# ishine/usdm

Measured on AMD Instinct MI355X. Metric: end-to-end real-time factor + LLM tokens/sec, 10 s utterance, 7B TP=1/8, higher is better.
Workload: dtype bf16; 1 GPU; full pipeline, one 10 s utterance: XLS-R tokenizer -> Mistral-7B (3 greedy rounds) -> Token-Voicebox 63 NFE (Heun, CFG, 3 s prompt) -> BigVGAN; wave_samples=160000, mel_frames=861, output_samples=220416, parallelism=tp1 (LLM) + replicas, tp_comm=none, voicebox=replica (CFG batch 2 on every rank)

## Files before the change

### include/usdm_hip.h

```cpp
#ifndef USDM_HIP_H_
#define USDM_HIP_H_
#include <stdint.h>

#ifdef __cplusplus
extern "C" {
#endif

typedef void* usdm_stream_t;

enum { USDM_BF16 = 0, USDM_F32 = 1 };
enum { USDM_ACT_NONE = 0, USDM_ACT_GELU = 1, USDM_ACT_SWIGLU = 3, USDM_ACT_TANH = 4, USDM_ACT_LOGCLAMP = 5  };
enum { USDM_EPI_PLAIN = 0, USDM_EPI_QKV_HEADS = 1 };

const char* usdm_last_error(void);
int usdm_abi_version(void);

typedef struct usdm_gemm_args {
  int32_t dtype;
  int32_t M, N;
  int32_t taps, Kc;
  const void* A;
  int64_t lda;
  int32_t rowsA;
  int32_t a_row_mul, a_row_off, a_row_step;
  int64_t a_tap_stride;
  const void* W;
  int64_t ldw;
  int32_t groups, batch;
  int64_t a_gstride;
  int64_t w_gstride;
  int64_t a_bstride;
  int32_t c_gcol;
  int64_t c_bstride;
  const float* bias;
  float alpha;
  int32_t act;
  int32_t round_bf16;
  const void* residual;
  int32_t res_dtype;
  int64_t ldr;
  void* C32;
  void* C16;
  int64_t ldc;
  int32_t c_row_mul, c_row_off;
  int32_t transpose_out;
  int32_t epi;
  int32_t qkv_S, qkv_Spad, qkv_H, qkv_D;
  void *qkv_q, *qkv_k, *qkv_v;
  int32_t split_k; int64_t c_split_stride;
  float* stats_out;
  const float* ln_stats; int32_t ln_nt, ln_mode, ln_C; float ln_eps;
  const float* ln_c; const float* ln_gamma; const float* ln_beta;
  int32_t* ln_guard; float ln_guard_ratio;
  int32_t tile_sel;
} usdm_gemm_args;

int usdm_gemm(const usdm_gemm_args* args, usdm_stream_t stream);
int usdm_gemm_tile_for(const usdm_gemm_args* args);

typedef struct usdm_norm_args {
  const void* x; int32_t x_dtype; int64_t ldx;
  const void* res; int32_t res_dtype; int64_t ldr;
  const float* gamma; const float* beta; float eps;
  int32_t rows, C;
  int32_t rms, act, round_bf16, premask;
  const int32_t* valid_len; int32_t rows_per_batch;
  void* out32; void* out16; int64_t ldo;
  void* sum32; void* sum16; int64_t lds;
  const float* res2; int32_t n_res2; int64_t res2_stride;
} usdm_norm_args;

int usdm_norm(const usdm_norm_args* args, usdm_stream_t stream);

typedef struct usdm_snake_args {
  const float* x; int64_t ldx;
  int32_t T, C, Creal, L;
  const float* alpha; const float* beta; int32_t logscale;
  float fup[12]; float fdn[12];
  float* out32; void* out16; int64_t ldo;
} usdm_snake_args;
int usdm_aa_snake(const usdm_snake_args* args, usdm_stream_t stream);

int usdm_sum3_scale(const float* a, const float* b, const float* c, float scale, int64_t n,
                    float* out32, void* out16_bf16, usdm_stream_t stream);

int usdm_cf_to_cl(const float* x, int32_t B, int32_t C, int32_t T, int32_t Cpad, float scale, float shift,
                  float* out32, void* out16_bf16, usdm_stream_t stream);

typedef struct usdm_attn_args {
  int32_t mode, dh, B, Hq, Hkv, Sq, Skv, Skv_alloc, q_pos0, alibi_col0_zero;
  float scale;
  int32_t head_order;
  const void* q; int64_t q_bs, q_hs, q_rs;
  const void* k; int64_t k_bs, k_hs, k_rs;
  const void* vt; int64_t v_bs, v_hs, v_ds;
  void* o; int64_t o_bs, o_rs;
  const int32_t* kv_len;
  const float* slopes;
  int32_t window;
  int32_t variant;
} usdm_attn_args;
int usdm_attention(const usdm_attn_args* args, usdm_stream_t stream);

typedef struct usdm_vb_input_args {
  const int64_t* ids;
  const float* y;
  const float* cond;
  const void* table;
  int32_t B_in, dup, S, E, F, null_id, use_cond;
  void* out; int64_t ldo;
  int32_t out_dtype;
} usdm_vb_input_args;
int usdm_vb_build_input(const usdm_vb_input_args* args, usdm_stream_t stream);

int usdm_softmax_alibi(float* x, int32_t rows, int32_t rows_per_batch, int32_t nheads, int32_t n, int32_t npad, int64_t ldrow,
                       int32_t ldseg, const float* slopes, const int32_t* kv_len, int32_t col0_zero, usdm_stream_t stream);

int usdm_vb_time_token(const float* t, int32_t t_stride, const float* freqs, int32_t Bx, int32_t H,
                       int64_t rows_per_batch, float* h32, void* h16_bf16, usdm_stream_t stream);

typedef struct usdm_vb_solver_args {
  const float* vout;
  const float* z; float* v1; const float* eps; const float* cond;
  float* z_in; float* z_commit; float* t_cur;
  int32_t B, F, S, P, cfg, mode, t_count;
  float gs, dt, c_eps, c_cond, t_next;
} usdm_vb_solver_args;
int usdm_vb_solver_step(const usdm_vb_solver_args* args, usdm_stream_t stream);

int usdm_mask_time(float* x32, void* x16_bf16, int32_t B, int32_t T, int32_t C, int32_t layout, const int32_t* valid_len,
                   int32_t off, usdm_stream_t stream);

int usdm_copy_bytes(void* dst, const void* src, int64_t nbytes, usdm_stream_t stream);

int usdm_process_unit(const int64_t* units, int32_t n, int32_t rep, int32_t hop, int64_t* out, int32_t nframes,
                      usdm_stream_t stream);

typedef struct usdm_gemv_args {
  const void* W; int64_t ldw; int32_t N, K;
  const void* x;
  const float* norm_w; float eps;
  int32_t act, round_bf16;
  const void* residual;
  void* y16; float* y32;
  const uint8_t* ban; float* part_val; int32_t* part_idx;
  int32_t idx_offset;
  const float* x_delta; void* x_out;
  const int32_t* skip;
  const struct usdm_p2p_dev* p2p; int32_t p2p_site, p2p_mode;
  const float* mrg_pm; const float* mrg_pl; const float* mrg_po; int32_t mrg_ns;
  unsigned long long* cmb_gran; int32_t* cmb_err; int32_t cmb_timeout_ms;
  int32_t resident;
} usdm_gemv_args;
int usdm_gemv(const usdm_gemv_args* args, usdm_stream_t stream);
int usdm_gemv_nblocks(int32_t N, int32_t act);

int usdm_gemv_threads(const usdm_gemv_args* args);

typedef struct usdm_gemv_batch_args {
  usdm_gemv_args g;
  int32_t nb;
  int64_t x_bs, y_bs, res_bs;
  int32_t part_bs;
  int32_t form;
  float* ks_part; int32_t* ks_cnt; int64_t ks_part_floats;
} usdm_gemv_batch_args;
int64_t usdm_gemv_batch_ks_floats(int32_t N, int32_t K);
int usdm_gemv_batch(const usdm_gemv_batch_args* args, usdm_stream_t stream);

typedef struct usdm_gemv_fp8_args {
  usdm_gemv_batch_args b;
  const int8_t* row_exp;
} usdm_gemv_fp8_args;
int usdm_gemv_fp8(const usdm_gemv_fp8_args* args, usdm_stream_t stream);
int usdm_gemv_fp8_mfma(const usdm_gemv_fp8_args* args, usdm_stream_t stream);
int usdm_dequant_fp8(const void* q, const int8_t* row_exp, int32_t N, int32_t K, int64_t ldq, void* out, int64_t ldo,
                     usdm_stream_t stream);
int usdm_sizeof_gemv_fp8_args(void);

typedef struct usdm_gemv_mxfp4_args {
  usdm_gemv_batch_args b;
  const uint8_t* scales;
  int64_t lds;
} usdm_gemv_mxfp4_args;
int usdm_gemv_mxfp4(const usdm_gemv_mxfp4_args* args, usdm_stream_t stream);
int usdm_dequant_mxfp4(const void* codes, int64_t ldw, const uint8_t* scales, int64_t lds, int32_t N, int32_t K, void* out,
                       int64_t ldo, usdm_stream_t stream);
int usdm_sizeof_gemv_mxfp4_args(void);

typedef struct usdm_decode_state {
  int32_t* next_token;
  int32_t* out_tokens;
  int32_t* step;
  int32_t* pos;
  int32_t max_out, id_offset, advance_pos;
  int32_t batch;
  int32_t* done; const int32_t* eos;
} usdm_decode_state;
int usdm_argmax_final(const float* part_val, const int32_t* part_idx, int32_t nparts,
                      const usdm_decode_state* st, const void* embed_table_bf16, int32_t Hd, void* h_out_bf16,
                      usdm_stream_t stream);
int usdm_argmax_final_seg(const float* part_val, const int32_t* part_idx, int32_t nparts, int32_t nseg, int64_t seg_stride,
                          const usdm_decode_state* st, const void* embed_table, int32_t Hd, void* h_out, usdm_stream_t stream);

typedef struct usdm_sample_params {
  float temperature; int32_t top_k; float top_p;
  float min_p;
  uint64_t seed;
} usdm_sample_params;
typedef struct usdm_sample_args {
  const float* logits; int32_t V;
  float temperature; int32_t top_k; float top_p;
  uint64_t seed;
  float* probs_out;
  const usdm_sample_params* dev_params;
  int64_t logits_bs;
  float min_p;
} usdm_sample_args;
int usdm_sample_final(const usdm_sample_args* args, const usdm_decode_state* st, const void* embed_table_bf16, int32_t Hd,
                      void* h_out_bf16, usdm_stream_t stream);
int usdm_sample_final_seg(const usdm_sample_args* args, int32_t nseg, int64_t seg_stride, int32_t seg_len, const usdm_decode_state* st,
                          const void* embed_table_bf16, int32_t Hd, void* h_out_bf16, usdm_stream_t stream);

typedef struct usdm_logprob_args {
  const float* logits; int32_t V; int32_t K;
  int64_t logits_bs;
  float* tok_lp; int32_t* tok_rank; int32_t* top_id; float* top_lp;
  int64_t tok_bs, top_bs;
  int32_t* count;
} usdm_logprob_args;
int usdm_logprobs(const usdm_logprob_args* args, const usdm_decode_state* st, usdm_stream_t stream);
int usdm_logprobs_seg(const usdm_logprob_args* args, int32_t nseg, int64_t seg_stride, int32_t seg_len, const usdm_decode_state* st,
                      usdm_stream_t stream);
int usdm_sizeof_logprob_args(void);

typedef struct usdm_prompt_logprob_args {
  const float* logits; int32_t V; int32_t K;
  int64_t logits_bs;
  const int64_t* ids;
  int32_t n_ids;
  int32_t row0, rows;
  float* tok_lp; int32_t* tok_rank; int32_t* top_id; float* top_lp;
} usdm_prompt_logprob_args;
int usdm_prompt_logprobs(const usdm_prompt_logprob_args* args, usdm_stream_t stream);
int usdm_prompt_logprobs_seg(const usdm_prompt_logprob_args* args, int32_t nseg, int64_t seg_stride, int32_t seg_len,
                             usdm_stream_t stream);
int usdm_sizeof_prompt_logprob_args(void);

typedef struct usdm_penalty_params { float repetition, frequency, presence; int32_t reserved; } usdm_penalty_params;
typedef struct usdm_penalty_args {
  float* logits; int32_t V;
  int64_t logits_bs;
  int32_t* table;
  int64_t table_bs;
  const usdm_penalty_params* dev_params;
  int32_t* count;
} usdm_penalty_args;
int usdm_penalize(const usdm_penalty_args* args, const usdm_decode_state* st, usdm_stream_t stream);
int usdm_penalize_seg(const usdm_penalty_args* args, int32_t nseg, int64_t seg_stride, int32_t seg_len, const usdm_decode_state* st,
                      usdm_stream_t stream);
int usdm_penalty_params_init(usdm_penalty_params* out, float repetition, float frequency, float presence);
int usdm_sizeof_penalty_args(void);
int usdm_sizeof_penalty_params(void);

typedef struct usdm_logit_edit_params { int32_t ngram, prompt_len, n_bias, reserved; } usdm_logit_edit_params;
typedef struct usdm_logit_edit_args {
  float* logits; int32_t V;
  int64_t logits_bs;
  const usdm_logit_edit_params* dev_params;
  const int32_t* bias_id; const float* bias_val;
  int32_t bias_max;
  int64_t bias_bs;
  const int32_t* prompt;
  int32_t prompt_max;
  int64_t prompt_bs;
} usdm_logit_edit_args;
int usdm_logit_edit(const usdm_logit_edit_args* args, const usdm_decode_state* st, usdm_stream_t stream);
int usdm_logit_edit_seg(const usdm_logit_edit_args* args, int32_t nseg, int64_t seg_stride, int32_t seg_len, const usdm_decode_state* st,
                        usdm_stream_t stream);
int usdm_sizeof_logit_edit_args(void);
int usdm_sizeof_logit_edit_params(void);

#define USDM_BEAM_MAX_KC 32
typedef struct usdm_beam_args {
  const float* logits; int32_t V;
  int64_t logits_bs;
  float* score;
  int32_t* parent;
  int32_t nlive, n_eos;
  const int32_t* eos;
  float* log_score; int32_t* log_token; int32_t* log_parent;
  int32_t log_rows;
  float* cand_score; int32_t* cand_index;
} usdm_beam_args;
int usdm_beam_step(const usdm_beam_args* args, const usdm_decode_state* st, const void* embed_table_bf16, int32_t Hd, void* h_out_bf16,
                   usdm_stream_t stream);
int usdm_sizeof_beam_args(void);

typedef struct usdm_kv_reorder_args {
  void* base[4]; int64_t slot_bytes[4]; int32_t row_bytes[4];
  int32_t n_arrays, nblk, ctx_max, B;
  const int32_t* parent; const int32_t* lo; const int32_t* pos;
} usdm_kv_reorder_args;
int usdm_kv_reorder(const usdm_kv_reorder_args* args, usdm_stream_t stream);
int usdm_sizeof_kv_reorder_args(void);

int usdm_embed_rows(const void* table, const int64_t* ids, const int32_t* next_token, int32_t n, int32_t Hd,
                    void* out, usdm_stream_t stream);

typedef struct usdm_rope_args {
// ... 145 lines not shown
```

### usdm_amd/csrc/gemv_launch.h

```cpp
#pragma once
#include "gemv_common.h"

namespace {
struct gemv_sel { int rw, nwv; bool glu; int grid; int res; };

static int gemv_pick_rw(int nout, bool glu) {
  const int ncand = glu ? 2 : 4;
  const int cands[4] = {glu ? 2 : 4, glu ? 1 : 3, 2, 1};
  int best = cands[ncand - 1];
  double best_score = -1.0;
  for (int c = 0; c < ncand; ++c) {
    const int rw = cands[c];
    const int blocks = cdiv(nout, 4 * rw);
    const double eff = (blocks / 256.0) / (double)((blocks + 255) / 256);
    if (blocks >= 1024 && eff >= 0.9) return rw;
    const double score = eff * (blocks >= 512 ? 1.0 : 0.5 + blocks / 1024.0);
    if (score > best_score) { best_score = score; best = rw; }
  }
  return best;
}

static gemv_sel gemv_select(const usdm_gemv_args& a, bool batched) {
  const bool glu = a.act == USDM_ACT_SWIGLU;
  const int nout = glu ? a.N / 2 : a.N;
  const int rows_per_cu = nout % 256 == 0 ? nout / 256 : 0;
  const gemv_sel wide16{1, 16, false, 256}, wide12{2, 12, false, 256};
  if (!batched && (a.mrg_po || a.p2p_mode)) return rows_per_cu == 16 ? wide16 : gemv_sel{1, 4, false, cdiv(nout, 4)};
  if (!glu && !a.part_val && rows_per_cu == 16) return wide16;
  if (!glu && !a.part_val && rows_per_cu == 24) return wide12;
  if (!batched && glu && (a.resident != 0 || (nout % 14 == 0 && (nout / 14) % 512 == 0)))
    return gemv_sel{2, 7, true, cdiv(nout, 14), a.resident < 0 ? 0 : a.resident > 0 ? a.resident : 0x7fffffff};
  const int rw = a.part_val ? 4 : gemv_pick_rw(nout, glu);
  return gemv_sel{rw, 4, glu, cdiv(nout, 4 * rw)};
}

enum { GEMV_PLAIN = 1, GEMV_BATCH = 2, GEMV_MRG = 4, GEMV_CMB = 8 };
#define USDM_GEMV_SHAPES(X)                                   \
  X(1, false, 16, GEMV_PLAIN | GEMV_BATCH | GEMV_MRG | GEMV_CMB) \
  X(2, false, 12, GEMV_PLAIN | GEMV_BATCH)                    \
  X(2, true, 7, GEMV_PLAIN)                                   \
  X(4, false, 4, GEMV_PLAIN | GEMV_BATCH)                     \
  X(3, false, 4, GEMV_PLAIN | GEMV_BATCH)                     \
  X(2, false, 4, GEMV_PLAIN | GEMV_BATCH)                     \
  X(1, false, 4, GEMV_PLAIN | GEMV_BATCH | GEMV_MRG)          \
  X(2, true, 4, GEMV_PLAIN | GEMV_BATCH)                      \
  X(1, true, 4, GEMV_PLAIN | GEMV_BATCH)
template <int FORM, class LAUNCH>
static bool gemv_dispatch(const gemv_sel& s, LAUNCH&& launch) {
#define USDM_GEMV_CASE(RW, GLU, NWV, FORMS)                                      \
  if constexpr (((FORMS) & FORM) != 0)                                           \
    if (s.rw == RW && s.glu == GLU && s.nwv == NWV) {                            \
      launch(gemv_ic<RW>{}, gemv_ic<GLU>{}, gemv_ic<NWV>{});                     \
      return true;                                                               \
    }
  USDM_GEMV_SHAPES(USDM_GEMV_CASE)
#undef USDM_GEMV_CASE
  return false;
}

static int gemv_no_instantiation(const gemv_sel& s) {
  usdm_set_error("%s: no instantiation for %d rows per wave, GLU %d, %d waves", __FILE__, s.rw, (int)s.glu, s.nwv);
  return 1;
}

static int gemv_check_shape(const char* who, const usdm_gemv_args& a, const char* x_noun) {
  USDM_CHECK_ARG(a.N > 0 && a.K > 0 && a.K % 8 == 0 && a.ldw % 8 == 0 && a.ldw >= a.K, "%s: bad N/K/ldw", who);
  USDM_CHECK_ARG(a.K <= 16384, "%s: K too large for the LDS-resident %s", who, x_noun);
  USDM_CHECK_ARG(a.act != USDM_ACT_SWIGLU || a.N % 32 == 0, "%s: swiglu needs N %% 32 == 0", who);
  return 0;
}
static int gemv_check_outputs(const char* who, const usdm_gemv_args& a) {
  USDM_CHECK_ARG(a.y16 || a.y32 || a.part_val, "%s: no output", who);
  USDM_CHECK_ARG(!a.part_val || (a.part_idx && a.act != USDM_ACT_SWIGLU), "%s: part_idx missing / lm_head mode is not GLU", who);
  return 0;
}
}
```

### usdm_amd/csrc/llm_k.hip

```cpp
#include "common.h"
#include <stdlib.h>
#include <utility>
#include "../../include/usdm_hip.h"
#include "gemv_launch.h"
#include "attn_merge.h"
#include "p2p.h"
#include "pick_commit.h"

#ifndef USDM_GEMV_X_FIRST
#define USDM_GEMV_X_FIRST 1
#endif
#ifndef USDM_GEMV_RES_PREFETCH
#define USDM_GEMV_RES_PREFETCH 1
#endif
namespace {
#ifdef USDM_GEMV_TRACE
__device__ unsigned long long g_gemv_trace[8192 * 8];
#define GTR(i) do { if (threadIdx.x == 0 && blockIdx.x < 8192) g_gemv_trace[blockIdx.x * 8 + (i)] = wall_clock64(); } while (0)
#else
#define GTR(i) do { } while (0)
#endif


template <int RW, bool GLU, int NWV, bool MRG = false, bool P2P = false, bool CMB = false, bool FP8 = false, class... FMT>
__global__ __launch_bounds__(NWV * 64) void gemv_kernel(const usdm_gemv_args a, FMT... fmt) {
  typedef typename gemv_fmt<FP8>::wvec wvec;
  constexpr bool MX4 = gemv_is_mx4<FMT...>::value;
  static_assert((FP8 || MX4) == (sizeof...(FMT) == 1) && !(FP8 && MX4), "FP8 takes the row exponents, MXFP4 the block scales");
  static_assert(!(FP8 || MX4) || (!MRG && !P2P && !CMB), "the FP8 / MXFP4 weight formats have the plain single-GPU forms only");
  constexpr int NTH = NWV * 64;
  constexpr int NR = GLU ? 2 * RW : RW;
  constexpr int UNR = gemv_ring_depth(NR, FP8, MX4);
  extern __shared__ __attribute__((aligned(16))) char smem[];
  bf16_t* xs = (bf16_t*)smem;
  __shared__ float red[NWV];
  __shared__ float sv[NWV];
  __shared__ int si[NWV];
  const int tid = threadIdx.x, lane = tid & 63, wave = tid >> 6;
  const int skipv = a.skip ? *a.skip : 0;
  unsigned p2p_epoch = 0u;
  bool p2p_failed = false;
  if constexpr (P2P) { p2p_epoch = p2p_load_epoch(a.p2p); p2p_failed = p2p_load_err(a.p2p) != 0u; }
  GTR(0);
  const int K = a.K;
  const int Kpad = (K + 511) & ~511;
  const int nit = Kpad >> 9;

  const int rows_per_block = NWV * RW;
  const int ob = blockIdx.x * rows_per_block + wave * RW;
  const wvec* wp[NR];
  float wsc[NR];
  const unsigned* wsp[MX4 ? NR : 1];
#pragma unroll
  for (int j = 0; j < NR; ++j) {
    int r;
    if (GLU) {
      const int o = ob + (j % RW);
      r = (o >> 4) * 32 + (o & 15) + (j >= RW ? 16 : 0);
    } else {
      r = ob + j;
    }
    r = r < a.N ? r : a.N - 1;
    if constexpr (FP8) {
      wp[j] = (const wvec*)((const uint8_t*)a.W + (int64_t)r * a.ldw) + lane;
      wsc[j] = fp8_row_scale(gemv_row_exp(fmt...)[r]);
    } else if constexpr (MX4) {
      const gemv_mx4 m = gemv_mx4_fmt(fmt...);
      wp[j] = (const u32x4*)((const uint8_t*)a.W + (int64_t)r * a.ldw) + lane;
      wsp[j] = (const unsigned*)(m.scales + (int64_t)r * m.lds) + (lane >> 2);
    } else {
      wp[j] = (const u32x4*)((const bf16_t*)a.W + (int64_t)r * a.ldw) + lane;
    }
  }
  const int ngr = (nit + 3) >> 2;
  const bool tail_ok = ((nit - 1) << 9) + lane * 8 < K;
  bool active = true;
  if (a.part_val && a.ban) {
    const int wb = blockIdx.x * rows_per_block;
    bool wg_active = false;
    for (int r = wb; r < wb + rows_per_block && r < a.N; ++r) wg_active |= (a.ban[r] == 0);
    if (!wg_active) {
      if (tid == 0) { a.part_val[blockIdx.x] = -INFINITY; a.part_idx[blockIdx.x] = 0x7fffffff; }
      if (a.y32 && tid < rows_per_block && wb + tid < a.N) a.y32[wb + tid] = -INFINITY;
      return;
    }
    active = false;
#pragma unroll
    for (int j = 0; j < NR; ++j)
      if (ob + j < a.N) active |= (a.ban[ob + j] == 0);
    active = __builtin_amdgcn_readfirstlane(active);
  }
  auto wload = [&](int j, int it) -> wvec {
    if (!active) return wvec{};
    const wvec* p = (it == nit - 1 && !tail_ok) ? wp[j] - lane : wp[j] + it * 64;
    return __builtin_nontemporal_load(p);
  };
  unsigned short resraw[GLU ? 1 : NR];
  if constexpr (!GLU && USDM_GEMV_RES_PREFETCH) {
    const bf16_t* rbase = a.residual ? (const bf16_t*)a.residual : (const bf16_t*)a.W;
#pragma unroll
    for (int j = 0; j < NR; ++j) resraw[j] = rbase[min(ob + j, a.N - 1)];
  }
  constexpr bool EARLY = USDM_GEMV_X_FIRST && !CMB && !MRG;
  const int i0 = tid * 8;
  u32x4 x0 = {0u, 0u, 0u, 0u}, ge0v = x0, ge1v = x0;
  if constexpr (EARLY) {
    const int ic = min(i0, K - 8);
    const float* gp0 = a.norm_w ? a.norm_w + ic : (const float*)a.x;
    const float* gp1 = a.norm_w ? gp0 + 4 : gp0;
    asm volatile("global_load_dwordx4 %0, %1, off" : "=v"(x0) : "v"((const bf16_t*)a.x + ic) : "memory");
    asm volatile("global_load_dwordx4 %0, %1, off" : "=v"(ge0v) : "v"(gp0) : "memory");
    asm volatile("global_load_dwordx4 %0, %1, off" : "=v"(ge1v) : "v"(gp1) : "memory");
  }
  wvec ring[NR][UNR];
  unsigned rsc[MX4 ? NR : 1][MX4 ? UNR : 1];
#pragma unroll
  for (int u = 0; u < UNR; ++u)
#pragma unroll
    for (int j = 0; j < NR; ++j) {
      if constexpr (MX4) {
        const int g = u < ngr ? u : 0;
        ring[j][u] = __builtin_nontemporal_load(wp[j] + g * 64);
        rsc[j][u] = __builtin_nontemporal_load(wsp[j] + g * 16);
      } else {
        const bool real = active && u < nit;
        const wvec* p = real ? ((u == nit - 1 && !tail_ok) ? wp[j] - lane : wp[j] + u * 64) : wp[j] - lane;
        ring[j][u] = __builtin_nontemporal_load(p);
      }
    }
  GTR(1);
  if constexpr (EARLY) {
    constexpr int NY = (MX4 ? 2 : 1) * UNR * NR;
    asm volatile("s_waitcnt vmcnt(%3)" : "+v"(x0), "+v"(ge0v), "+v"(ge1v) : "n"(NY));
  }
  if (skipv) return;
  const float4 ge0 = __builtin_bit_cast(float4, ge0v), ge1 = __builtin_bit_cast(float4, ge1v);
  const bf16_t* xg = (const bf16_t*)a.x;
  auto with_delta = [&](u32x4 v, int i, bool publish) -> u32x4 {
    if (a.x_delta) {
      const float4 d0 = *(const float4*)(a.x_delta + i), d1 = *(const float4*)(a.x_delta + i + 4);
      const float dl[8] = {d0.x, d0.y, d0.z, d0.w, d1.x, d1.y, d1.z, d1.w};
#pragma unroll
      for (int e = 0; e < 4; ++e)
        v[e] = pack_bf2(bf2f(v[e] & 0xffff) + round_bf(dl[2 * e]), bf2f(v[e] >> 16) + round_bf(dl[2 * e + 1]));
      if (publish && a.x_out && blockIdx.x == 0) *(u32x4*)((bf16_t*)a.x_out + i) = v;
    }
    return v;
  };
  auto ldx = [&](int i, bool publish) -> u32x4 { return with_delta(*(const u32x4*)(xg + i), i, publish); };
  const int iloop = EARLY ? i0 + NTH * 8 : i0;
  if (a.norm_w) {
    float ss = 0.f;
    u32x4 v0 = x0;
    if constexpr (EARLY) {
      if (i0 < K) {
        v0 = with_delta(x0, i0, false);
#pragma unroll
        for (int e = 0; e < 4; ++e) {
          const float lo = bf2f(v0[e] & 0xffff), hi = bf2f(v0[e] >> 16);
          ss += lo * lo + hi * hi;
        }
      }
    }
    for (int i = iloop; i < K; i += NTH * 8) {
      const u32x4 v = ldx(i, false);
#pragma unroll
// ... 309 lines not shown
  const int i0 = tid * 8;
  u32x4 x0 = {0u, 0u, 0u, 0u}, ge0v = x0, ge1v = x0;
  {
    const int ic = min(i0, K - 8);
    const float* gp0 = a.norm_w ? a.norm_w + ic : (const float*)a.x;
    const float* gp1 = a.norm_w ? gp0 + 4 : gp0;
    asm volatile("global_load_dwordx4 %0, %1, off" : "=v"(x0) : "v"((const bf16_t*)a.x + ic) : "memory");
    asm volatile("global_load_dwordx4 %0, %1, off" : "=v"(ge0v) : "v"(gp0) : "memory");
    asm volatile("global_load_dwordx4 %0, %1, off" : "=v"(ge1v) : "v"(gp1) : "memory");
  }
  u32x4 ring[NR][UNR];
  if constexpr (TPW > 0) {
    static_assert(NIT == 0 || (NIT >= UNR && NIT % UNR == 0), "slot u = iteration u of every tile");
    gemv_for<UNR>([&](auto U) { gemv_for<NR>([&](auto J) { aload(ring[J.value][U.value], wp[J.value], U); }); });
  } else {
#pragma unroll
    for (int u = 0; u < UNR; ++u)
#pragma unroll
      for (int j = 0; j < NR; ++j) ring[j][u] = u < nit ? wload(wp[j], u) : __builtin_nontemporal_load((const u32x4*)wp[j]);
  }
  GTR(1);
  asm volatile("s_waitcnt vmcnt(%3)" : "+v"(x0), "+v"(ge0v), "+v"(ge1v) : "n"(UNR * NR));
  if (skipv) return;
  const float4 ge0 = __builtin_bit_cast(float4, ge0v), ge1 = __builtin_bit_cast(float4, ge1v);
  const bf16_t* xg = (const bf16_t*)a.x;
  const int iloop = i0 + NTH * 8;
  if (a.norm_w) {
    float ss = 0.f;
    if (i0 < K) {
#pragma unroll
      for (int e = 0; e < 4; ++e) {
        const float lo = bf2f(x0[e] & 0xffff), hi = bf2f(x0[e] >> 16);
        ss += lo * lo + hi * hi;
      }
    }
    for (int i = iloop; i < K; i += NTH * 8) {
      const u32x4 v = *(const u32x4*)(xg + i);
#pragma unroll
      for (int e = 0; e < 4; ++e) {
        const float lo = bf2f(v[e] & 0xffff), hi = bf2f(v[e] >> 16);
        ss += lo * lo + hi * hi;
      }
    }
    ss = wave_sum(ss);
    if (lane == 0) red[wave] = ss;
    __syncthreads();
    float tot = 0.f;
#pragma unroll
    for (int w = 0; w < NWV; ++w) tot += red[w];
    const float rstd = rsqrtf(tot / (float)K + a.eps);
    auto normed = [&](u32x4 v, float4 g0, float4 g1) -> u32x4 {
      const float gw[8] = {g0.x, g0.y, g0.z, g0.w, g1.x, g1.y, g1.z, g1.w};
      u32x4 o;
#pragma unroll
      for (int e = 0; e < 4; ++e) {
        const float lo = bf2f(v[e] & 0xffff), hi = bf2f(v[e] >> 16);
        o[e] = pack_bf2(round_bf(round_bf(lo * rstd) * gw[2 * e]), round_bf(round_bf(hi * rstd) * gw[2 * e + 1]));
      }
      return o;
    };
    if (i0 < Kpad) *(u32x4*)(xs + i0) = i0 < K ? normed(x0, ge0, ge1) : u32x4{0, 0, 0, 0};
    for (int i = iloop; i < Kpad; i += NTH * 8) {
      u32x4 o = {0, 0, 0, 0};
      if (i < K) o = normed(*(const u32x4*)(xg + i), *(const float4*)(a.norm_w + i), *(const float4*)(a.norm_w + i + 4));
      *(u32x4*)(xs + i) = o;
    }
  } else {
    if (i0 < Kpad) *(u32x4*)(xs + i0) = i0 < K ? x0 : u32x4{0, 0, 0, 0};
    for (int i = iloop; i < Kpad; i += NTH * 8) {
      u32x4 v = {0, 0, 0, 0};
      if (i < K) v = *(const u32x4*)(xg + i);
      *(u32x4*)(xs + i) = v;
    }
  }
  __syncthreads();
  GTR(2);

  float acc[NR];
  const char* wn[NR];
  auto finish = [&](int t) {
#pragma unroll
    for (int j = 0; j < NR; ++j) acc[j] = wave_sum(acc[j]);
    if (t < 4) GTR(3 + t);
    if (lane == 0) {
      const int ob = (blockIdx.x + t * gridDim.x) * TILE + wave * RW;
#pragma unroll
      for (int j = 0; j < RW; ++j) {
        const int o = ob + j;
        if (2 * o >= a.N) continue;
        const float r = gemv_swiglu_value(acc[j], acc[j + RW], a.round_bf16);
        if (a.y16) ((bf16_t*)a.y16)[o] = f2bf(r);
        if (a.y32) a.y32[o] = r;
      }
    }
#pragma unroll
    for (int j = 0; j < NR; ++j) wp[j] = wn[j];
  };
  if constexpr (TPW > 0) {
    u32x4 xv = *(const u32x4*)(xs + lane * 8);
    gemv_for<TPW>([&](auto T) {
      constexpr int t = decltype(T)::value;
      constexpr bool has_next = t + 1 < TPW;
#pragma unroll
      for (int j = 0; j < NR; ++j) {
        acc[j] = 0.f;
        wn[j] = has_next ? row_ptr(t + 1, j) : wp[j];
      }
      gemv_for<NIT>([&](auto IT) {
        constexpr int it = decltype(IT)::value, u = it % UNR;
        constexpr bool refill = it + UNR < NIT || has_next;
        const u32x4 xn = *(const u32x4*)(xs + (((it + 1) % NIT) * 64 + lane) * 8);
        gemv_for<NR>([&](auto J) {
          constexpr int j = decltype(J)::value;
          constexpr int younger = refill ? NR * UNR - 1 : NR * UNR - 1 - ((it - (NIT - UNR)) * NR + j);
          asm volatile("s_waitcnt vmcnt(%1)" : "+v"(ring[j][u]) : "n"(younger) : "memory");
          acc[j] = dot8(ring[j][u], xv, acc[j]);
          if constexpr (it + UNR < NIT) aload(ring[j][u], wp[j], gemv_ic<it + UNR>{});
          else if constexpr (has_next) aload(ring[j][u], wn[j], gemv_ic<u>{});
        });
        xv = xn;
      });
      finish(t);
    });
  } else {
    const int ntiles = (a.N / 2 + TILE - 1) / TILE;
    const int ntl = (ntiles - (int)blockIdx.x + (int)gridDim.x - 1) / (int)gridDim.x;
    for (int t = 0; t < ntl; ++t) {
      const bool has_next = t + 1 < ntl;
#pragma unroll
      for (int j = 0; j < NR; ++j) {
        acc[j] = 0.f;
        wn[j] = has_next ? row_ptr(t + 1, j) : wp[j];
      }
      for (int it0 = 0; it0 < nit; it0 += UNR) {
#pragma unroll
        for (int u = 0; u < UNR; ++u) {
          const int it = it0 + u;
          if (it < nit) {
            const u32x4 xv = *(const u32x4*)(xs + (it * 64 + lane) * 8);
#pragma unroll
            for (int j = 0; j < NR; ++j) {
              acc[j] = dot8(ring[j][u], xv, acc[j]);
              const bool own = it + UNR < nit;
              if (own || has_next) ring[j][u] = wload(own ? wp[j] : wn[j], own ? it + UNR : u);
            }
          }
        }
      }
      finish(t);
    }
  }
}

__global__ void argmax_final_kernel(const float* pv, const int* pi, int nparts, int nseg, int64_t seg_stride, usdm_decode_state st,
                                    const bf16_t* E, int Hd, bf16_t* h_out) {
  __shared__ float sv[256];
  __shared__ int si[256];
  __shared__ int s_tok;
  const int b = blockIdx.x;
  if (st.done && st.done[b]) return;
  pv += (int64_t)b * nparts; pi += (int64_t)b * nparts;
  float bv = -INFINITY;
  int bi = PICK_NO_ID;
  for (int sg = 0; sg < nseg; ++sg)
    for (int i = threadIdx.x; i < nparts; i += 256) {
      const float v = pv[sg * seg_stride + i];
      const int id = pi[sg * seg_stride + i];
      if (pick_better(v, id, bv, bi)) { bv = v; bi = id; }
    }
  pick_block_best<256>(sv, si, bv, bi);
  if (threadIdx.x == 0) {
    const int tok = (si[0] == PICK_NO_ID ? 0 : si[0]) + st.id_offset;
    pick_commit(st, b, st.step[b], tok);
    s_tok = tok;
  }
  if (E) {
    __syncthreads();
    pick_embed_row<256>(E, s_tok, Hd, h_out + (int64_t)b * Hd);
  }
}

__global__ void embed_kernel(const bf16_t* E, const int64_t* ids, const int* next_token, int n, int Hd, bf16_t* out) {
  const int r = blockIdx.x;
  const int64_t id = ids ? ids[r] : (int64_t)(*next_token);
  const u32x4* src = (const u32x4*)(E + id * Hd);
  u32x4* dst = (u32x4*)(out + (int64_t)r * Hd);
  for (int i = threadIdx.x; i < Hd / 8; i += blockDim.x) dst[i] = src[i];
}

__global__ void residual_add_kernel(bf16_t* h, const float* delta, int n) {
  const int i = blockIdx.x * blockDim.x + threadIdx.x;
  if (i < n) h[i] = f2bf(bf2f(h[i]) + round_bf(delta[i]));
}
}

static int gemv_resident_count(const void* kern, int nth, size_t lds, int* out) {
  static thread_local const void* c_kern = nullptr;
  static thread_local int c_dev = -1, c_n = 0;
  static thread_local size_t c_lds = 0;
  int dev = 0;
  USDM_HIP(hipGetDevice(&dev));
  if (kern != c_kern || dev != c_dev || lds != c_lds) {
    int ncu = 0, per = 0;
    USDM_HIP(hipDeviceGetAttribute(&ncu, hipDeviceAttributeMultiprocessorCount, dev));
    USDM_HIP(hipOccupancyMaxActiveBlocksPerMultiprocessor(&per, kern, nth, lds));
    USDM_CHECK_ARG(ncu > 0 && per > 0, "usdm_gemv: the resident form does not fit a CU (%zu bytes of LDS)", lds);
    c_kern = kern; c_dev = dev; c_lds = lds; c_n = ncu * per;
  }
  *out = c_n;
  return 0;
}

static int gemv_launch_resident(const usdm_gemv_args& a, const gemv_sel& s, size_t lds, hipStream_t st, bool* launched) {
  *launched = false;
  if (a.x_delta) return 0;
  constexpr int RW = 2, NWV = 7;
  auto straight = gemv_resident_kernel<RW, NWV, 2, 8>;
  auto generic = gemv_resident_kernel<RW, NWV, 0, 0>;
  const int ntiles = s.grid;
  int n = 0;
  if (int rc = gemv_resident_count((const void*)straight, NWV * 64, lds, &n)) return rc;
  int grid = min(min(n, s.res), ntiles);
  if (grid == ntiles) return 0;
  if (a.K == 8 * 512 && ntiles == 2 * grid) {
    hipLaunchKernelGGL(straight, dim3(grid), dim3(NWV * 64), lds, st, a);
  } else {
    if (int rc = gemv_resident_count((const void*)generic, NWV * 64, lds, &n)) return rc;
    grid = min(min(n, s.res), ntiles);
    if (grid == ntiles) return 0;
    hipLaunchKernelGGL(generic, dim3(grid), dim3(NWV * 64), lds, st, a);
  }
  *launched = true;
  USDM_LAUNCH_CHECK();
  return 0;
}

template <int FORM, bool MRG, bool P2P, bool CMB, bool FP8, class... FMT>
static int gemv_launch(const usdm_gemv_args& a, hipStream_t st, FMT... fmt) {
  const size_t lds = (size_t)((a.K + 511) & ~511) * 2;
  const gemv_sel s = gemv_select(a, false);
  if constexpr (FORM == GEMV_PLAIN && !FP8 && sizeof...(FMT) == 0) {
    if (s.res > 0) {
      bool launched = false;
      if (int rc = gemv_launch_resident(a, s, lds, st, &launched)) return rc;
      if (launched) return 0;
    }
  }
  const bool found = gemv_dispatch<FORM>(s, [&](auto RW, auto GLU, auto NWV) {
    constexpr int nwv = decltype(NWV)::value;
    hipLaunchKernelGGL((gemv_kernel<decltype(RW)::value, decltype(GLU)::value != 0, nwv, MRG, P2P, CMB, FP8, FMT...>), dim3(s.grid),
                       dim3(nwv * 64), lds, st, a, fmt...);
  });
  if (!found) return gemv_no_instantiation(s);
  USDM_LAUNCH_CHECK();
  return 0;
}

extern "C" int usdm_gemv(const usdm_gemv_args* pa, usdm_stream_t stream) {
  USDM_CHECK_ARG(pa && pa->W && (pa->x || pa->mrg_po), "usdm_gemv: null args");
  const usdm_gemv_args& a = *pa;
  if (int rc = gemv_check_shape("usdm_gemv", a, "input vector")) return rc;
  if (int rc = gemv_check_outputs("usdm_gemv", a)) return rc;
  const bool glu = a.act == USDM_ACT_SWIGLU;
  USDM_CHECK_ARG(!a.norm_w || a.K % 8 == 0, "usdm_gemv: K");
  USDM_CHECK_ARG(!a.x_out || (a.x_delta && a.x_out != a.x), "usdm_gemv: x_out needs x_delta and must not alias x");
  USDM_CHECK_ARG(!a.mrg_po || (a.mrg_pm && a.mrg_pl && a.mrg_ns >= 1 && a.mrg_ns <= 64 && a.K % 128 == 0 && !a.norm_w && !a.x_delta),
                 "usdm_gemv: merged-attention input needs pm/pl/po, 1 <= splits <= 64, K a multiple of 128, no norm / x_delta");
  USDM_CHECK_ARG(a.p2p_mode >= 0 && a.p2p_mode <= 2, "usdm_gemv: p2p_mode");
  USDM_CHECK_ARG(!a.p2p_mode || (a.p2p && a.p2p_site >= 0 && a.act == USDM_ACT_NONE && !a.part_val && a.residual && a.y16),
                 "usdm_gemv: the fused all-reduce needs a plain row-parallel projection with residual + y16");
  const int nout = glu ? a.N / 2 : a.N;
  hipStream_t st = (hipStream_t)stream;
  if (a.cmb_gran) {
    USDM_CHECK_ARG(a.mrg_po && a.mrg_pm && a.mrg_pl && a.mrg_ns >= 1 && a.mrg_ns <= 64 && !a.p2p_mode && !glu && !a.part_val && !a.norm_w && !a.x_delta &&
                       nout % 256 == 0 && nout / 256 == 16 && a.K % 128 == 0 && a.K / 128 <= 256,
                   "usdm_gemv: cmb_gran needs the mrg_* partials, a plain 4096-output projection and K / 128 <= 256 heads");
    return gemv_launch<GEMV_CMB, false, false, true, false>(a, st);
  }
  if (a.mrg_po || a.p2p_mode) {
    USDM_CHECK_ARG(!glu && !a.part_val, "usdm_gemv: merged-attention input / fused all-reduce are for plain projections");
    if (a.mrg_po && a.p2p_mode) return gemv_launch<GEMV_MRG, true, true, false, false>(a, st);
    if (a.mrg_po) return gemv_launch<GEMV_MRG, true, false, false, false>(a, st);
    return gemv_launch<GEMV_MRG, false, true, false, false>(a, st);
  }
  return gemv_launch<GEMV_PLAIN, false, false, false, false>(a, st);
}

int usdm_gemv_fp8_batch_launch(const usdm_gemv_fp8_args* pa, hipStream_t st);

extern "C" int usdm_gemv_fp8(const usdm_gemv_fp8_args* pa, usdm_stream_t stream) {
  USDM_CHECK_ARG(pa && pa->b.g.W && pa->b.g.x && pa->row_exp, "usdm_gemv_fp8: null args");
  const usdm_gemv_args& a = pa->b.g;
  USDM_CHECK_ARG(pa->b.nb >= 1 && pa->b.nb <= 4 && (pa->b.form == 0 || pa->b.form == -1),
                 "usdm_gemv_fp8: 1..4 sequences on the VALU form (the matrix-core form has no FP8 weights)");
  USDM_CHECK_ARG(!a.p2p && !a.p2p_mode && !a.mrg_po && !a.cmb_gran && !a.x_delta && !a.x_out,
                 "usdm_gemv_fp8: p2p / merged-attention input / cmb_gran / x_delta are not supported with FP8 weights");
  USDM_CHECK_ARG(((uintptr_t)a.W & 7) == 0, "usdm_gemv_fp8: bad N/K/ldw");
  if (int rc = gemv_check_shape("usdm_gemv_fp8", a, "input vector")) return rc;
  if (int rc = gemv_check_outputs("usdm_gemv_fp8", a)) return rc;
  hipStream_t st = (hipStream_t)stream;
  if (pa->b.nb > 1) return usdm_gemv_fp8_batch_launch(pa, st);
  return gemv_launch<GEMV_PLAIN, false, false, false, true>(a, st, pa->row_exp);
}

namespace {
__global__ __launch_bounds__(256) void dequant_fp8_kernel(const uint8_t* q, const int8_t* row_exp, int K, int64_t ldq, bf16_t* out,
                                                          int64_t ldo) {
  const int r = blockIdx.x;
  const float s = fp8_row_scale(row_exp[r]);
  const uint8_t* qr = q + (int64_t)r * ldq;
  bf16_t* orow = out + (int64_t)r * ldo;
  for (int i = threadIdx.x * 8; i < K; i += 256 * 8) {
    const u32x2 w = __builtin_nontemporal_load((const u32x2*)(qr + i));
    *(u32x4*)(orow + i) = fp8x8_to_bf16x8(w, s);
  }
}
}

extern "C" int usdm_dequant_fp8(const void* q, const int8_t* row_exp, int32_t N, int32_t K, int64_t ldq, void* out, int64_t ldo,
                                usdm_stream_t stream) {
  USDM_CHECK_ARG(q && row_exp && out, "usdm_dequant_fp8: null args");
  USDM_CHECK_ARG(N > 0 && K > 0 && K % 8 == 0 && ldq >= K && ldq % 8 == 0 && ldo >= K && ldo % 8 == 0, "usdm_dequant_fp8: bad N/K/ldq/ldo");
  USDM_CHECK_ARG(((uintptr_t)q & 7) == 0 && ((uintptr_t)out & 15) == 0, "usdm_dequant_fp8: q must be 8-byte, out 16-byte aligned");
  hipLaunchKernelGGL(dequant_fp8_kernel, dim3(N), dim3(256), 0, (hipStream_t)stream, (const uint8_t*)q, row_exp, K, ldq, (bf16_t*)out, ldo);
  USDM_LAUNCH_CHECK();
  return 0;
}
extern "C" int usdm_sizeof_gemv_fp8_args(void) { return (int)sizeof(usdm_gemv_fp8_args); }

int usdm_gemv_mxfp4_batch_launch(const usdm_gemv_mxfp4_args* pa, hipStream_t st);

extern "C" int usdm_gemv_mxfp4(const usdm_gemv_mxfp4_args* pa, usdm_stream_t stream) {
  USDM_CHECK_ARG(pa && pa->b.g.W && pa->b.g.x && pa->scales, "usdm_gemv_mxfp4: null args");
  const usdm_gemv_args& a = pa->b.g;
  USDM_CHECK_ARG(pa->b.nb >= 1 && pa->b.nb <= 4 && (pa->b.form == 0 || pa->b.form == -1),
                 "usdm_gemv_mxfp4: 1..4 sequences on the VALU form (the matrix-core form has no MXFP4 weights)");
  USDM_CHECK_ARG(!a.p2p && !a.p2p_mode && !a.mrg_po && !a.mrg_pm && !a.mrg_pl && !a.cmb_gran && !a.x_delta && !a.x_out,
                 "usdm_gemv_mxfp4: p2p / merged-attention input / cmb_gran / x_delta are not supported with MXFP4 weights");
  USDM_CHECK_ARG(!a.part_val && !a.part_idx && !a.ban && !a.y32, "usdm_gemv_mxfp4: the lm_head mode (part_val / ban / y32) is not supported with MXFP4 weights");
  USDM_CHECK_ARG(a.N > 0 && a.K > 0 && a.K % 32 == 0 && a.K <= 16384, "usdm_gemv_mxfp4: K must be a multiple of 32, at most 16384");
  USDM_CHECK_ARG(a.ldw % 1024 == 0 && 2 * a.ldw >= a.K && pa->lds % 64 == 0 && 32 * pa->lds >= a.K,
                 "usdm_gemv_mxfp4: ldw (bytes) must hold whole groups of 1024 bytes and lds whole groups of 64 bytes covering K");
  USDM_CHECK_ARG(((uintptr_t)a.W & 15) == 0 && ((uintptr_t)pa->scales & 3) == 0 && ((uintptr_t)a.x & 15) == 0,
                 "usdm_gemv_mxfp4: codes and x must be 16-byte, scales 4-byte aligned");
  USDM_CHECK_ARG(a.act != USDM_ACT_SWIGLU || a.N % 32 == 0, "usdm_gemv_mxfp4: swiglu needs N %% 32 == 0");
  if (int rc = gemv_check_outputs("usdm_gemv_mxfp4", a)) return rc;
  hipStream_t st = (hipStream_t)stream;
  if (pa->b.nb > 1) return usdm_gemv_mxfp4_batch_launch(pa, st);
  return gemv_launch<GEMV_PLAIN, false, false, false, false>(a, st, gemv_mx4{pa->scales, pa->lds});
}

namespace {
__global__ __launch_bounds__(256) void dequant_mxfp4_kernel(const uint8_t* codes, int64_t ldw, const uint8_t* scales, int64_t lds, int K,
                                                            bf16_t* out, int64_t ldo) {
  const int r = blockIdx.x;
  const u32x4* cr = (const u32x4*)(codes + (int64_t)r * ldw);
  const unsigned* sr = (const unsigned*)(scales + (int64_t)r * lds);
  bf16_t* orow = out + (int64_t)r * ldo;
  const int npiece = ((K + 2047) >> 11) * 64;
  for (int p = threadIdx.x; p < npiece; p += 256) {
    const int g = p >> 6, L = p & 63;
    const u32x4 w = __builtin_nontemporal_load(cr + p);
    const unsigned sc = sr[g * 16 + (L >> 2)];
    const int e = g * 2048 + L * 8;
    if (e < K) *(u32x4*)(orow + e) = mx4x8_to_bf16x8<0>(w[0], sc);
    if (e + 512 < K) *(u32x4*)(orow + e + 512) = mx4x8_to_bf16x8<1>(w[1], sc);
    if (e + 1024 < K) *(u32x4*)(orow + e + 1024) = mx4x8_to_bf16x8<2>(w[2], sc);
    if (e + 1536 < K) *(u32x4*)(orow + e + 1536) = mx4x8_to_bf16x8<3>(w[3], sc);
  }
}
}

extern "C" int usdm_dequant_mxfp4(const void* codes, int64_t ldw, const uint8_t* scales, int64_t lds, int32_t N, int32_t K, void* out,
                                  int64_t ldo, usdm_stream_t stream) {
  USDM_CHECK_ARG(codes && scales && out, "usdm_dequant_mxfp4: null args");
  USDM_CHECK_ARG(N > 0 && K > 0 && K % 32 == 0 && ldo >= K && ldo % 8 == 0, "usdm_dequant_mxfp4: bad N/K/ldo");
  USDM_CHECK_ARG(ldw % 1024 == 0 && 2 * ldw >= K && lds % 64 == 0 && 32 * lds >= K,
                 "usdm_dequant_mxfp4: ldw (bytes) must hold whole groups of 1024 bytes and lds whole groups of 64 bytes covering K");
  USDM_CHECK_ARG(((uintptr_t)codes & 15) == 0 && ((uintptr_t)scales & 3) == 0 && ((uintptr_t)out & 15) == 0,
                 "usdm_dequant_mxfp4: codes and out must be 16-byte, scales 4-byte aligned");
  hipLaunchKernelGGL(dequant_mxfp4_kernel, dim3(N), dim3(256), 0, (hipStream_t)stream, (const uint8_t*)codes, ldw, scales, lds, K,
                     (bf16_t*)out, ldo);
  USDM_LAUNCH_CHECK();
  return 0;
}
extern "C" int usdm_sizeof_gemv_mxfp4_args(void) { return (int)sizeof(usdm_gemv_mxfp4_args); }

#ifdef USDM_GEMV_TRACE
extern "C" int usdm_dbg_gemv_trace(unsigned long long* host, int n) {
  return (int)hipMemcpyFromSymbol(host, HIP_SYMBOL(g_gemv_trace), sizeof(unsigned long long) * n);
}
#endif

extern "C" int usdm_gemv_nblocks(int32_t N, int32_t act) { return cdiv(N, 16); }

extern "C" int usdm_gemv_threads(const usdm_gemv_args* pa) { return 64 * gemv_select(*pa, false).nwv; }

extern "C" int usdm_argmax_final_seg(const float* part_val, const int32_t* part_idx, int32_t nparts, int32_t nseg, int64_t seg_stride,
                                     const usdm_decode_state* st, const void* embed_table, int32_t Hd, void* h_out,
                                     usdm_stream_t stream) {
  USDM_CHECK_ARG(part_val && part_idx && nparts > 0 && st && st->next_token && st->out_tokens && st->step && st->pos,
                 "usdm_argmax_final: bad args");
  USDM_CHECK_ARG(nseg >= 1 && (nseg == 1 || seg_stride >= (int64_t)nparts * (st->batch > 1 ? st->batch : 1)), "usdm_argmax_final_seg: segments overlap");
  USDM_CHECK_ARG(!embed_table || (h_out && Hd > 0 && Hd % 8 == 0), "usdm_argmax_final: embedding output missing");
  USDM_CHECK_ARG(st->batch >= 0 && st->batch <= 64, "usdm_argmax_final: batch");
  hipLaunchKernelGGL(argmax_final_kernel, dim3(st->batch > 1 ? st->batch : 1), dim3(256), 0, (hipStream_t)stream, part_val, part_idx, nparts, nseg,
                     seg_stride, *st, (const bf16_t*)embed_table, Hd, (bf16_t*)h_out);
  USDM_LAUNCH_CHECK();
  return 0;
}
extern "C" int usdm_argmax_final(const float* part_val, const int32_t* part_idx, int32_t nparts,
                                 const usdm_decode_state* st, const void* embed_table, int32_t Hd, void* h_out,
                                 usdm_stream_t stream) {
  return usdm_argmax_final_seg(part_val, part_idx, nparts, 1, 0, st, embed_table, Hd, h_out, stream);
}

extern "C" int usdm_embed_rows(const void* table, const int64_t* ids, const int32_t* next_token, int32_t n, int32_t Hd,
                               void* out, usdm_stream_t stream) {
  USDM_CHECK_ARG(table && out && (ids || next_token) && n > 0, "usdm_embed_rows: bad args");
  USDM_CHECK_ARG(Hd % 8 == 0, "usdm_embed_rows: Hd=%d must be a multiple of 8 (16-byte row copies)", Hd);
  hipLaunchKernelGGL(embed_kernel, dim3(n), dim3(256), 0, (hipStream_t)stream, (const bf16_t*)table, ids, next_token, n, Hd,
                     (bf16_t*)out);
  USDM_LAUNCH_CHECK();
  return 0;
}

extern "C" int usdm_residual_add(void* h, const float* delta, int32_t n, usdm_stream_t stream) {
  USDM_CHECK_ARG(h && delta && n > 0, "usdm_residual_add: bad args");
  hipLaunchKernelGGL(residual_add_kernel, dim3(cdiv(n, 256)), dim3(256), 0, (hipStream_t)stream, (bf16_t*)h, delta, n);
  USDM_LAUNCH_CHECK();
  return 0;
}
extern "C" int usdm_sizeof_gemv_args(void) { return (int)sizeof(usdm_gemv_args); }
extern "C" int usdm_sizeof_decode_state(void) { return (int)sizeof(usdm_decode_state); }
```

Measured before the change: 5.245 x real-time (output audio s / wall s).

## Add streaming GEMV kernel for the K=14336 down projection

Adds a dedicated GEMV kernel for the MLP down projection (K=14336, no GLU, no norm). Each wave owns one output row and streams its weight row through an unrolled register ring, using non-temporal loads with explicit vmcnt waits. x is staged once into LDS, and the residual add is fused into the epilogue. The selector routes matching shapes to this kernel, which is meant to keep more weight loads in flight than the generic wide16 path. In exchange it hardcodes NIT=28 and bypasses the resident and generic paths for this shape.

```diff
diff --git a/include/usdm_hip.h b/include/usdm_hip.h
--- a/include/usdm_hip.h
+++ b/include/usdm_hip.h
@@ -156,6 +156,7 @@
 int usdm_gemv_nblocks(int32_t N, int32_t act);
 
 int usdm_gemv_threads(const usdm_gemv_args* args);
+int usdm_gemv_streams(const usdm_gemv_args* args);
 
 typedef struct usdm_gemv_batch_args {
   usdm_gemv_args g;
diff --git a/usdm_amd/csrc/gemv_launch.h b/usdm_amd/csrc/gemv_launch.h
--- a/usdm_amd/csrc/gemv_launch.h
+++ b/usdm_amd/csrc/gemv_launch.h
@@ -2,7 +2,7 @@
 #include "gemv_common.h"
 
 namespace {
-struct gemv_sel { int rw, nwv; bool glu; int grid; int res; };
+struct gemv_sel { int rw, nwv; bool glu; int grid; int res; bool stream; };
 
 static int gemv_pick_rw(int nout, bool glu) {
   const int ncand = glu ? 2 : 4;
@@ -26,7 +26,9 @@
   const int rows_per_cu = nout % 256 == 0 ? nout / 256 : 0;
   const gemv_sel wide16{1, 16, false, 256}, wide12{2, 12, false, 256};
   if (!batched && (a.mrg_po || a.p2p_mode)) return rows_per_cu == 16 ? wide16 : gemv_sel{1, 4, false, cdiv(nout, 4)};
-  if (!glu && !a.part_val && rows_per_cu == 16) return wide16;
+  const bool stream = !batched && !glu && !a.part_val && a.K == 14336 && !a.norm_w && !a.x_delta && a.resident >= 0;
+  if (stream && a.resident > 0) return gemv_sel{1, 16, false, cdiv(nout, 16), 0, true};
+  if (!glu && !a.part_val && rows_per_cu == 16) return gemv_sel{1, 16, false, 256, 0, stream};
   if (!glu && !a.part_val && rows_per_cu == 24) return wide12;
   if (!batched && glu && (a.resident != 0 || (nout % 14 == 0 && (nout / 14) % 512 == 0)))
     return gemv_sel{2, 7, true, cdiv(nout, 14), a.resident < 0 ? 0 : a.resident > 0 ? a.resident : 0x7fffffff};
diff --git a/usdm_amd/csrc/llm_k.hip b/usdm_amd/csrc/llm_k.hip
--- a/usdm_amd/csrc/llm_k.hip
+++ b/usdm_amd/csrc/llm_k.hip
@@ -12,6 +12,9 @@
 #endif
 #ifndef USDM_GEMV_RES_PREFETCH
 #define USDM_GEMV_RES_PREFETCH 1
+#endif
+#ifndef USDM_GEMV_DOWN_UNR
+#define USDM_GEMV_DOWN_UNR 8
 #endif
 namespace {
 #ifdef USDM_GEMV_TRACE
@@ -627,6 +630,65 @@
   }
 }
 
+template <int NIT, int UNR>
+__global__ __launch_bounds__(1024) __attribute__((amdgpu_waves_per_eu(4))) void gemv_stream_kernel(const usdm_gemv_args a) {
+  constexpr int NWV = 16, NTH = NWV * 64, K = NIT * 512;
+  static_assert(NIT >= UNR && UNR >= 1 && K <= 2 * NTH * 8, "a full first ring; a thread stages at most two pieces of x");
+  extern __shared__ __attribute__((aligned(16))) char smem[];
+  bf16_t* xs = (bf16_t*)smem;
+  const int tid = threadIdx.x, lane = tid & 63, wave = tid >> 6;
+  int skipv = a.skip ? *a.skip : 0;
+  GTR(0);
+  const int ob = blockIdx.x * NWV + wave;
+  const int urow = min((int)blockIdx.x * NWV + __builtin_amdgcn_readfirstlane(wave), a.N - 1);
+  const char* wp = (const char*)((const bf16_t*)a.W + (int64_t)urow * a.ldw);
+  const unsigned voff = lane * 16;
+  auto aload = [&](u32x4& dst, const char* p, auto IT) {
+    constexpr int it = decltype(IT)::value;
+    const unsigned vo = voff + (it >> 2) * 4096u;
+    asm volatile("global_load_dwordx4 %0, %1, %2 offset:%3 nt" : "=v"(dst) : "v"(vo), "s"(p), "n"((it & 3) * 1024) : "memory");
+  };
+  const bf16_t* rbase = a.residual ? (const bf16_t*)a.residual : (const bf16_t*)a.W;
+  const unsigned short resraw = rbase[min(ob, a.N - 1)];
+  const int i0 = tid * 8, i1 = i0 + NTH * 8;
+  u32x4 x0, x1;
+  asm volatile("global_load_dwordx4 %0, %1, off" : "=v"(x0) : "v"((const bf16_t*)a.x + min(i0, K - 8)) : "memory");
+  asm volatile("global_load_dwordx4 %0, %1, off" : "=v"(x1) : "v"((const bf16_t*)a.x + min(i1, K - 8)) : "memory");
+  u32x4 ring[UNR];
+  gemv_for<UNR>([&](auto U) { aload(ring[U.value], wp, U); });
+  GTR(1);
+  asm volatile("s_waitcnt vmcnt(%3)" : "+v"(x0), "+v"(x1), "+s"(skipv) : "n"(UNR));
+  if (skipv) return;
+  if (i0 < K) *(u32x4*)(xs + i0) = x0;
+  if (i1 < K) *(u32x4*)(xs + i1) = x1;
+  __syncthreads();
+  GTR(2);
+
+  float acc = 0.f;
+  u32x4 xv = *(const u32x4*)(xs + lane * 8);
+  gemv_for<NIT>([&](auto IT) {
+    constexpr int it = decltype(IT)::value, u = it % UNR;
+    constexpr int younger = it + UNR < NIT ? UNR - 1 : NIT - 1 - it;
+    const u32x4 xn = *(const u32x4*)(xs + (((it + 1) % NIT) * 64 + lane) * 8);
+    asm volatile("s_waitcnt vmcnt(%1)" : "+v"(ring[u]) : "n"(younger) : "memory");
+    acc = dot8(ring[u], xv, acc);
+    if constexpr (it + UNR < NIT) aload(ring[u], wp, gemv_ic<it + UNR>{});
+    xv = xn;
+  });
+  acc = wave_sum(acc);
+  GTR(3);
+
+  if (lane != 0 || ob >= a.N) return;
+  float v = acc;
+  if (a.round_bf16) v = round_bf(v);
+  if (a.residual) {
+    v += bf2f(resraw);
+    if (a.round_bf16) v = round_bf(v);
+  }
+  if (a.y16) ((bf16_t*)a.y16)[ob] = f2bf(v);
+  if (a.y32) a.y32[ob] = v;
+}
+
 __global__ void argmax_final_kernel(const float* pv, const int* pi, int nparts, int nseg, int64_t seg_stride, usdm_decode_state st,
                                     const bf16_t* E, int Hd, bf16_t* h_out) {
   __shared__ float sv[256];
@@ -715,6 +777,11 @@
   const size_t lds = (size_t)((a.K + 511) & ~511) * 2;
   const gemv_sel s = gemv_select(a, false);
   if constexpr (FORM == GEMV_PLAIN && !FP8 && sizeof...(FMT) == 0) {
+    if (s.stream) {
+      hipLaunchKernelGGL((gemv_stream_kernel<28, USDM_GEMV_DOWN_UNR>), dim3(s.grid), dim3(1024), lds, st, a);
+      USDM_LAUNCH_CHECK();
+      return 0;
+    }
     if (s.res > 0) {
       bool launched = false;
       if (int rc = gemv_launch_resident(a, s, lds, st, &launched)) return rc;
@@ -870,6 +937,7 @@
 extern "C" int usdm_gemv_nblocks(int32_t N, int32_t act) { return cdiv(N, 16); }
 
 extern "C" int usdm_gemv_threads(const usdm_gemv_args* pa) { return 64 * gemv_select(*pa, false).nwv; }
+extern "C" int usdm_gemv_streams(const usdm_gemv_args* pa) { return gemv_select(*pa, false).stream ? 1 : 0; }
 
 extern "C" int usdm_argmax_final_seg(const float* part_val, const int32_t* part_idx, int32_t nparts, int32_t nseg, int64_t seg_stride,
                                      const usdm_decode_state* st, const void* embed_table, int32_t Hd, void* h_out,
```

Result: faster. 5.400 x real-time (output audio s / wall s) (median of 6 runs) (+3.0%).
